# shanghong/Multiband-RF-pulse-Design

Hardware: AMD Instinct MI355X
Metric: FIR designs/sec, n=512 taps m=16384 arbitrary-phase SOCP (fir_ap_cvx form) (higher is better)
Workload: dtype f64

## Files before the change

include/mbfir.h:

```cpp
#ifndef MBFIR_H
#define MBFIR_H

#ifdef __cplusplus
extern "C" {
#endif

#define MBFIR_SOLVED 0
#define MBFIR_INFEASIBLE 1
#define MBFIR_NUMERICAL 2
#define MBFIR_EARLY_FAIL 3
#define MBFIR_E_ARG (-1)
#define MBFIR_E_HIP (-2)
#define MBFIR_E_NODEVICE (-3)

typedef struct mbfir_ctx mbfir_ctx;

typedef struct mbfir_opts {
    int grid_m;
    int max_iter;
    double feastol;
    double abstol;
    double reltol;
    int refine;
    int verbose;
// ... 21 lines not shown
    double chol_flop;
    int chol_launches;
    int builds;
    int dd_iters;
    int dd_kmax;
    int collectives;
    int lanes;
    int dd_form;
    double ms_cap;
    double cap_flop;
    double collective_bytes;
    int correctors;
    int correctors_taken;
    int gv_passes;
    int gtv_passes;
} mbfir_info;

typedef int (*mbfir_allreduce_fn)(void* buf, long count, int op, void* user);

int  mbfir_comm_unique_id(mbfir_ctx* ctx, char* id128);
int  mbfir_comm_init(mbfir_ctx* ctx, int nranks, int rank, const char* id128);
void mbfir_comm_destroy(mbfir_ctx* ctx);
int  mbfir_test_comm_allreduce(mbfir_ctx* ctx, double* v, long n, int op);

mbfir_ctx*  mbfir_create(int device_id);
void        mbfir_destroy(mbfir_ctx* ctx);
const char* mbfir_last_error(mbfir_ctx* ctx);
void        mbfir_default_opts(mbfir_opts* opts);
void        mbfir_set_allreduce(mbfir_ctx* ctx, mbfir_allreduce_fn fn, void* user);
const char* mbfir_version(void);
// ... 121 lines not shown
```

multiband-rf-pulse-design_amd/__init__.py:

```python
import ctypes as C
import os

import numpy as np

_HERE = os.path.dirname(os.path.abspath(__file__))
LIB_PATH = os.path.join(_HERE, "libmbfir.so")

SOLVED, INFEASIBLE, NUMERICAL, EARLY_FAIL = 0, 1, 2, 3
E_ARG, E_HIP, E_NODEVICE = -1, -2, -3


class MbfirError(RuntimeError):
    pass


class Opts(C.Structure):
    _fields_ = [("grid_m", C.c_int), ("max_iter", C.c_int), ("feastol", C.c_double),
                ("abstol", C.c_double), ("reltol", C.c_double), ("refine", C.c_int),
                ("verbose", C.c_int), ("shard_rank", C.c_int), ("shard_size", C.c_int),
                ("dense_trig", C.c_int), ("ddkkt", C.c_int), ("lanes", C.c_int)]


class Info(C.Structure):
    _fields_ = [("status", C.c_int), ("iters", C.c_int), ("n_unknowns", C.c_int), ("n_rows", C.c_int),
                ("n_freq", C.c_int), ("n_lp", C.c_int), ("n_q3", C.c_int), ("n_big", C.c_int),
                ("pcost", C.c_double), ("dcost", C.c_double), ("gap", C.c_double), ("relgap", C.c_double),
                ("pres", C.c_double), ("dres", C.c_double),
                ("ms_assemble", C.c_double), ("ms_solve", C.c_double), ("ms_post", C.c_double),
                ("ms_total", C.c_double), ("ms_gram", C.c_double), ("ms_chol", C.c_double),
                ("gram_flop", C.c_double), ("gram_launches", C.c_int), ("lattice", C.c_int),
                ("chol_flop", C.c_double), ("chol_launches", C.c_int), ("builds", C.c_int),
                ("dd_iters", C.c_int), ("dd_kmax", C.c_int), ("collectives", C.c_int), ("lanes", C.c_int),
                ("dd_form", C.c_int), ("ms_cap", C.c_double), ("cap_flop", C.c_double),
                ("collective_bytes", C.c_double), ("correctors", C.c_int), ("correctors_taken", C.c_int),
                ("gv_passes", C.c_int), ("gtv_passes", C.c_int)]

    def as_dict(self):
        return {k: getattr(self, k) for k, _ in self._fields_}


class Job(C.Structure):
    _fields_ = [("which", C.c_int), ("n", C.c_int), ("nband", C.c_int), ("rc", C.c_int),
                ("f", C.POINTER(C.c_double)), ("a", C.POINTER(C.c_double)), ("d", C.POINTER(C.c_double)),
                ("params", C.c_double * 4), ("h_re", C.POINTER(C.c_double)), ("h_im", C.POINTER(C.c_double)),
                ("info", Info), ("z", C.POINTER(C.c_double)), ("z_cap", C.c_int), ("err", C.c_char * 128)]


class RemezJob(C.Structure):
    _fields_ = [("numtaps", C.c_int), ("nband", C.c_int), ("type", C.c_int), ("edges", C.POINTER(C.c_double)),
                ("desired", C.POINTER(C.c_double)), ("weight", C.POINTER(C.c_double)), ("h", C.POINTER(C.c_double)),
# ... 1005 lines not shown
```

multiband-rf-pulse-design_amd/csrc/api.cpp:

```cpp
#include "../../include/mbfir.h"
#include "program.h"
#include "pulse.h"
#include "solver.h"
#include <chrono>
#include <cmath>
#include <cstdio>
#include <algorithm>
#include <cstdlib>
#include <cstring>
#include <functional>
#include <atomic>
#include <condition_variable>
#include <map>
#include <mutex>
#include <memory>
#include <system_error>
#include <thread>

using namespace mbfir;

struct mbfir_ctx {
    std::unique_ptr<Solver> solver;
    int device = 0;
    std::vector<double> last_x;
// ... 49 lines not shown
    info->status = rc; info->iters = si.iters; info->n_unknowns = P.N();
    info->n_rows = si.n_rows; info->n_freq = si.n_freq;
    info->n_lp = P.l; info->n_q3 = P.nq3; info->n_big = P.big;
    info->pcost = si.pcost; info->dcost = si.dcost; info->gap = si.gap; info->relgap = si.relgap;
    info->pres = si.pres; info->dres = si.dres;
    info->ms_assemble = (t_asm - t0) + si.ms_assemble; info->ms_solve = si.ms_solve;
    info->ms_post = t_end - t_solved; info->ms_total = t_end - t0;
    info->ms_gram = si.ms_gram; info->ms_chol = si.ms_chol; info->gram_flop = si.gram_flop;
    info->gram_launches = si.lattice ? 0 : si.h_builds * (P.quad ? 3 : 1);
    info->lattice = si.lattice;
    info->chol_launches = si.chol_launches; info->chol_flop = si.chol_flop; info->builds = si.h_builds;
    info->dd_iters = si.dd_iters; info->dd_kmax = si.dd_kmax; info->lanes = si.lanes; info->collectives = si.collectives;
    info->collective_bytes = si.collective_bytes;
    info->ms_cap = si.ms_cap; info->cap_flop = si.cap_flop; info->dd_form = si.dd_iters > 0 ? si.dd_form : -1;
    info->correctors = si.correctors; info->correctors_taken = si.correctors_taken; info->gv_passes = si.gv_passes; info->gtv_passes = si.gtv_passes;
}

void taps_from_solution(Solver& solver, const TrigProgram& P, const std::vector<double>& x, int lane, double* h_re, double* h_im) {
    const int n = P.n;
    switch (P.which) {
        case DES_AP:
            solver.specfact_last(n, h_re, h_im, lane);
            break;
        case DES_LINPROG: {
            const int nh = P.nhalf;
            for (int i = 0; i < n; ++i) { h_re[i] = 0; h_im[i] = 0; }
            if (P.real_filter) {
                if (P.odd_filter) for (int k = 0; k < nh; ++k) { h_re[nh - 1 + k] = x[k]; h_re[nh - 1 - k] = x[k]; }
                else for (int k = 0; k < nh; ++k) { h_re[nh + k] = x[k]; h_re[nh - 1 - k] = x[k]; }
            } else if (P.odd_filter) {
// ... 757 lines not shown
```

multiband-rf-pulse-design_amd/csrc/solver.h:

```cpp
#pragma once
#include "program.h"
#include <stdexcept>
#include <string>
#include <vector>

namespace mbfir {

struct ShapeError : std::runtime_error {
    explicit ShapeError(const std::string& s) : std::runtime_error(s) {}
};
struct ResourceError : std::runtime_error {
    explicit ResourceError(const std::string& s) : std::runtime_error(s) {}
};

enum { ST_OPTIMAL = 0, ST_PRIMAL_INFEASIBLE = 1, ST_DUAL_INFEASIBLE = 2, ST_MAXIT = 3, ST_NUMERICAL = 4,
       ST_OPTIMAL_INACCURATE = 5 };

struct SolveOpts {
    int max_iter = 200;
    double feastol = 1e-8, abstol = 1e-10, reltol = 1e-8;
    int refine = 2;
    int verbose = 0;
    int shard_rank = 0, shard_size = 1;
    bool dense_trig = false;
// ... 5 lines not shown
struct SolveInfo {
    int status = 0, iters = 0, n_unknowns = 0, n_rows = 0, n_freq = 0;
    double pcost = 0, dcost = 0, gap = 0, relgap = 0, pres = 0, dres = 0;
    double ms_assemble = 0, ms_solve = 0, ms_gram = 0, ms_chol = 0, gram_flop = 0;
    int h_builds = 0;
    int chol_launches = 0;
    double chol_flop = 0;
    int dd_iters = 0, dd_kmax = 0;
    double ms_cap = 0, cap_flop = 0;
    int dd_form = 0;
    int collectives = 0;
    double collective_bytes = 0;
    int lanes = 1;
    int lattice = 0;
    int correctors = 0, correctors_taken = 0;
    int gv_passes = 0, gtv_passes = 0;
};

class Solver {
public:
    explicit Solver(int device);
    ~Solver();
    Solver(const Solver&) = delete;
    Solver& operator=(const Solver&) = delete;
    int solve(const TrigProgram& P, const SolveOpts& o, std::vector<double>& xout, SolveInfo& info);
    void solve_lanes(const std::vector<const TrigProgram*>& Ps, const SolveOpts& o, std::vector<std::vector<double>>& xouts,
                     std::vector<SolveInfo>& infos);
    static std::vector<long> shape_key(const TrigProgram& P, const SolveOpts& o);
    static int max_lanes(const TrigProgram& P, const SolveOpts& o);
    static void test_fold(const double* w, int Mf, int fold, long* out);
// ... 24 lines not shown
```

multiband-rf-pulse-design_amd/csrc/solver.hip:

```cpp
#include "dev_common.h"
#include <functional>
#include <mutex>
#include <thread>
#include "cone_dev.h"
#include "dd_dev.h"
#include "program.h"
#include "solver.h"
#include <algorithm>
#include <chrono>
#include <cmath>
#include <cstdlib>
#include <cstring>
#include <vector>

#include <dlfcn.h>
#include <rccl/rccl.h>

namespace mbfir {

struct RcclApi {
    ncclResult_t (*GetUniqueId)(ncclUniqueId*) = nullptr;
    ncclResult_t (*CommInitRank)(ncclComm_t*, int, ncclUniqueId, int) = nullptr;
    ncclResult_t (*CommDestroy)(ncclComm_t) = nullptr;
    ncclResult_t (*AllReduce)(const void*, void*, size_t, ncclDataType_t, ncclRedOp_t, ncclComm_t, hipStream_t) = nullptr;
// ... 443 lines not shown
            if (P.own)
            for (int q = P.c_ptr[j]; q < P.c_ptr[j + 1]; ++q) {
                const int r = P.c_rows[q];
                g += P.alpha[r] * val[(long)v * P.Rp + r];
            }
            if (F.bx) __hip_atomic_store(out + (long)v * P.LDV + j, g, __ATOMIC_RELAXED, __HIP_MEMORY_SCOPE_AGENT);
            else out[(long)v * P.LDV + j] = g;
        }
    }
    if (F.bx) gt_resid_tail<NV>(P, F, out, red);
}

constexpr int CHK = 64;

constexpr int SEGMAX = 128;
template <int NV>
__global__ __launch_bounds__(256) void k_trig_eval(DProg P, const double* __restrict__ vin, double* __restrict__ UU) {
    LANES(P, vin, UU);
    constexpr int NVVMAX = 2 * NV;
    __shared__ double2 cf[NVVMAX][SEGMAX];
    const int k = blockIdx.x * 256 + threadIdx.x, sg = blockIdx.y;
    const int m0 = sg * P.seg, m1 = min(m0 + P.seg, P.D1);
    const int NVV = P.quad ? 2 * NV : NV;
    for (int e = threadIdx.x; e < 2 * (m1 - m0); e += 256) {
        const int kind = e & 1, m = m0 + (e >> 1), le = kind * P.D1 + m;
        const int j = P.lat_col[le], qj = P.quad ? P.lat_qcol[le] : -1;
        const double sc = P.lat_scale[le], qs = P.quad ? P.lat_qscale[le] : 0.0;
#pragma unroll
        for (int q = 0; q < NV; ++q) {
            const double c1 = j >= 0 ? sc * vin[(long)q * P.LDV + j] : 0.0;
            if (kind) cf[q][e >> 1].y = c1; else cf[q][e >> 1].x = c1;
            if (P.quad) {
                const double c2 = qj >= 0 ? qs * vin[(long)q * P.LDV + qj] : 0.0;
                if (kind) cf[NV + q][e >> 1].y = c2; else cf[NV + q][e >> 1].x = c2;
            }
        }
    }
    __syncthreads();
    if (k >= P.nfold) return;
    const double4 sd4 = P.seed_eval[(long)sg * P.Mpad + k];
    double c = sd4.x, s = sd4.y;
    const double cw = sd4.z, sw = sd4.w;
    double ac[NVVMAX], as[NVVMAX];
#pragma unroll
    for (int v = 0; v < NVVMAX; ++v) ac[v] = as[v] = 0;
#pragma unroll 8
    for (int m = 0; m < m1 - m0; ++m) {
#pragma unroll
        for (int v = 0; v < NVVMAX; ++v)
            if (v < NVV) { const double2 x = cf[v][m]; ac[v] += x.x * c; as[v] += x.y * s; }
        const double cn = c * cw - s * sw;
        s = s * cw + c * sw;
        c = cn;
    }
    const int ip = P.fold_pos[k], in = P.fold_neg[k];
#pragma unroll
    for (int v = 0; v < NVVMAX; ++v)
        if (v < NVV) {
            double* u = UU + ((long)sg * NVV + v) * P.Mpad;
            if (ip >= 0) u[ip] = ac[v] + as[v];
            if (in >= 0) u[in] = ac[v] - as[v];
        }
}

__global__ void k_build_seeds_m(DProg P, double ka, int na, double kb, int nb, double4* __restrict__ seeds) {
    LANES(P, seeds);
    if (P.dims) { na = P.D1; nb = nb ? 2 * P.D1 - 1 : 0; }
    const double t0a = ka * P.tmin, t0b = kb * P.tmin;
    const int m = blockIdx.x * blockDim.x + threadIdx.x, ch = blockIdx.y;
    if (m >= na + nb || ch >= P.nchunk) return;
    const double t = m < na ? t0a + m : t0b + (m - na);
    double s, c, sd, cd;
    sincos(P.ch_w0[ch] * t, &s, &c);
    sincos(P.ch_dw[ch] * t, &sd, &cd);
    seeds[(long)ch * (na + nb) + m] = make_double4(c, s, cd, sd);
}
__global__ void k_build_seeds_e(DProg P, double4* __restrict__ seeds) {
    LANES(P, seeds);
    const int i = blockIdx.x * blockDim.x + threadIdx.x, sg = blockIdx.y;
    if (i >= P.nfold) return;
    const double w = P.wf[i];
    double s, c, sw, cw;
    sincos(w * (P.tmin + sg * P.seg), &s, &c);
    sincos(w, &sw, &cw);
    seeds[(long)sg * P.Mpad + i] = make_double4(c, s, cw, sw);
}

constexpr int CGRP = 4;
constexpr int MPTS = 256;
template <int NV, bool AGG>
__device__ __forceinline__ void freq_operands(const DProg& P, const double* __restrict__ src, int i, double (&out)[NV]) {
#pragma unroll
    for (int v = 0; v < NV; ++v) out[v] = 0;
    if (i < 0) return;
    if (AGG) {
        const int nv = P.quad ? NV / 2 : NV;
        for (int qq = P.f_ptr[i]; qq < P.f_ptr[i + 1]; ++qq) {
            const int r = P.f_rows[qq];
            const double al = P.alpha[r], be = P.beta[r];
#pragma unroll
            for (int v = 0; v < NV; ++v)
                if (v < nv) {
                    const double x = src[(long)v * P.Rp + r];
                    out[v] += al * x;
// ... 4 lines not shown
#pragma unroll
        for (int v = 0; v < NV; ++v) out[v] = src[(long)v * P.Mpad + i];
    }
}
template <int NV, bool AGG>
__global__ __launch_bounds__(256) void k_freq_fold(DProg P, const double* __restrict__ src, double2* __restrict__ out) {
    LANES(P, src, out);
    const int k = blockIdx.x * 256 + threadIdx.x;
    if (k >= P.nfold) return;
    double a[NV], b[NV];
    freq_operands<NV, AGG>(P, src, P.fold_pos[k], a);
    freq_operands<NV, AGG>(P, src, P.fold_neg[k], b);
#pragma unroll
    for (int v = 0; v < NV; ++v) out[(long)v * P.Mpad + k] = make_double2(a[v] + b[v], a[v] - b[v]);
}
template <int NV, bool FOLD = false>
__global__ __launch_bounds__(256) void k_trig_moments(DProg P, const double2* __restrict__ src, const double4* __restrict__ seeds,
                                                      int na, int nb, double* __restrict__ partial, const double* __restrict__ rows = nullptr) {
    if (!P.seeds_shared && blockIdx.z) seeds = reinterpret_cast<const double4*>(reinterpret_cast<const char*>(seeds) + (size_t)blockIdx.z * P.lane_bytes);
    LANES(P, src, partial, rows);
    if (P.dims) { na = P.D1; nb = nb ? 2 * P.D1 - 1 : 0; }
    __shared__ double2 pp[NV][CGRP][CHK];
    const int tid = threadIdx.x;
    const int ch0 = blockIdx.y * P.cgrp;
    for (int e = tid; e < P.cgrp * CHK; e += 256) {
        const int cc = e / CHK, q = e - cc * CHK, ch = ch0 + cc;
        const bool live = ch < P.nchunk && q < P.ch_count[ch < P.nchunk ? ch : 0];
        const int k = live ? P.ch_start[ch] + q : 0;
        if constexpr (FOLD) {
            double a[NV], b[NV];
            freq_operands<NV, true>(P, rows, live ? P.fold_pos[k] : -1, a);
            freq_operands<NV, true>(P, rows, live ? P.fold_neg[k] : -1, b);
#pragma unroll
            for (int v = 0; v < NV; ++v) pp[v][cc][q] = make_double2(a[v] + b[v], a[v] - b[v]);
        } else {
#pragma unroll
        for (int v = 0; v < NV; ++v) pp[v][cc][q] = live ? src[(long)v * P.Mpad + k] : make_double2(0.0, 0.0);
        }
    }
    __syncthreads();
    const int m = blockIdx.x * MPTS + tid;
    if (m >= na + nb) return;
    double ag[NV], as[NV];
#pragma unroll
    for (int v = 0; v < NV; ++v) ag[v] = as[v] = 0;
    for (int cl = 0; cl < P.cgrp; cl += 2) {
        const int cha = ch0 + cl, chb = cha + 1;
        if (cha >= P.nchunk) break;
        const bool two = cl + 1 < P.cgrp && chb < P.nchunk;
        const double4 sa = seeds[(long)cha * (na + nb) + m];
        const double4 sb = two ? seeds[(long)chb * (na + nb) + m] : make_double4(0.0, 0.0, 0.0, 0.0);
        double c0 = sa.x, s0 = sa.y, c1 = sb.x, s1 = sb.y;
        const int cnt = max(P.ch_count[cha], two ? P.ch_count[chb] : 0);
        const int clb = two ? cl + 1 : cl;
#pragma unroll 4
        for (int q = 0; q < cnt; ++q) {
#pragma unroll
            for (int v = 0; v < NV; ++v) {
                const double2 pa = pp[v][cl][q], pb = pp[v][clb][q];
                ag[v] += pa.x * c0; as[v] += pa.y * s0;
                ag[v] += pb.x * c1; as[v] += pb.y * s1;
            }
            const double n0 = c0 * sa.z - s0 * sa.w, n1 = c1 * sb.z - s1 * sb.w;
            s0 = s0 * sa.z + c0 * sa.w; s1 = s1 * sb.z + c1 * sb.w;
            c0 = n0; c1 = n1;
        }
    }
#pragma unroll
    for (int v = 0; v < NV; ++v) {
        partial[(((long)blockIdx.y * NV + v) * 2) * P.LDM + m] = ag[v];
        partial[(((long)blockIdx.y * NV + v) * 2 + 1) * P.LDM + m] = as[v];
    }
}

template <int NC>
__device__ __forceinline__ void block_partials(double vals[NC], double* __restrict__ part, bool is_max) {
    __shared__ double sh[17];
#pragma unroll
    for (int c = 0; c < NC; ++c) {
        double s = is_max ? block_max(vals[c], sh) : block_sum(vals[c], sh);
        if (threadIdx.x == 0) part[(long)blockIdx.x * NC + c] = s;
    }
}
__device__ __forceinline__ double fold_partials(const double* part, int nb, int nc, int c, bool is_max, double* sh) {
    double a = is_max ? -1e300 : 0.0;
    for (int b = threadIdx.x; b < nb; b += blockDim.x) {
// ... 1156 lines not shown
    bool corr_big = true;
    int test_cap_kp = 0;
    int ar_chunks = 0;
    int ar_overlap = 1;
    int cgrp = 4;
    int ddform = -1;
    bool dd_blockinv = true;
    bool hsolve = true;
    bool fuse = true;
    bool speculate = true;
    bool trace_host = false;
    int fold = -1;
    int chol_split = -1;
    bool poison = false;
    int test_lose_flag = -1;
};
static SolveSwitches read_switches() {
    SolveSwitches w;
    auto flag = [](const char* name, bool& v) { if (const char* ev = std::getenv(name)) v = std::atoi(ev) != 0; };
    auto number = [](const char* name, int& v) { if (const char* ev = std::getenv(name)) v = std::atoi(ev); };
    flag("MBFIR_CORRECTOR", w.corrector); flag("MBFIR_CORR_BIG", w.corr_big); flag("MBFIR_DD_BLOCKINV", w.dd_blockinv);
    flag("MBFIR_HSOLVE", w.hsolve); flag("MBFIR_FUSE", w.fuse); flag("MBFIR_SPECULATE", w.speculate); flag("MBFIR_POISON", w.poison);
    number("MBFIR_TEST_CAP_KP", w.test_cap_kp); number("MBFIR_AR_OVERLAP", w.ar_overlap);
    number("MBFIR_CHOL_SPLIT", w.chol_split); number("MBFIR_TEST_LOSE_FLAG", w.test_lose_flag);
    if (const char* ev = std::getenv("MBFIR_CGRP")) w.cgrp = std::max(1, std::min(CGRP, std::atoi(ev)));
    if (const char* ev = std::getenv("MBFIR_AR_CHUNKS")) w.ar_chunks = std::max(1, std::atoi(ev));
    if (const char* ev = std::getenv("MBFIR_DDFORM")) w.ddform = std::strcmp(ev, "dd") != 0 ? 1 : 0;
    if (const char* ev = std::getenv("MBFIR_FOLD")) w.fold = std::atoi(ev) != 0;
    w.trace_host = std::getenv("MBFIR_TRACE_HOST") != nullptr;
    return w;
}

struct LatticeInfo {
    bool ok = false;
    double tmin = 0;
    int D1 = 0;
    std::vector<int> lat, lat_col, lat_qcol, ch_start, ch_count;
    std::vector<double> lat_scale, lat_qscale, ch_w0, ch_dw;
    std::vector<int> fold_pos, fold_neg;
    std::vector<double> wf;
};
constexpr int CHUNK_LEN = 64;
static_assert(CHUNK_LEN <= CHK, "a chunk holds at most CHK frequencies");
// ... 216 lines not shown
    if (L.wall >= WALL_ITERS) return finish(ST_NUMERICAL);
    return best;
}

struct Solver::Impl {
    int device = 0;
    hipStream_t st = nullptr;
    int shard_rank = 0, shard_size = 1;
    int (*ar_fn)(void*, long, int, void*) = nullptr;
    void* ar_user = nullptr;
    double* RB = nullptr;
    ncclComm_t comm = nullptr;
    int comm_size = 0, comm_rank = 0;
    long n_collectives = 0;
    double collective_bytes = 0;
    long n_gv = 0, n_gtv = 0;
    void allreduce(double* buf, long count, int op, hipStream_t on = nullptr) {
        if (shard_size <= 1) return;
        if (!on) on = st;
        ++n_collectives;
        collective_bytes += 8.0 * double(count);
        if (comm) {
            ncclResult_t r = rccl().AllReduce(buf, buf, size_t(count), ncclDouble, op == 1 ? ncclMax : ncclSum, comm, on);
            if (r != ncclSuccess) throw HipError(std::string("ncclAllReduce: ") + (rccl().GetErrorString ? rccl().GetErrorString(r) : "failed"));
            return;
        }
        MBFIR_HIP(hipStreamSynchronize(on));
        if (!ar_fn || ar_fn(buf, count, op, ar_user) != 0) throw HipError("all-reduce hook failed");
    }
    hipEvent_t ev0 = nullptr, ev1 = nullptr;
// ... 122 lines not shown
        pend.clear();
        stage_lo = stage_hi = 0;
    }
    void memset_lanes(void* p, size_t bytes) {
        if ((bytes & 15) == 0 && (reinterpret_cast<size_t>(p) & 15) == 0 && (lane_bytes & 15) == 0)
            hipLaunchKernelGGL(k_zero_lanes, dim3(std::min<size_t>(2048, cdiv((long)(bytes / 16), 256)), nlanes), dim3(256), 0, st,
                               reinterpret_cast<double2*>(p), bytes / 16, lane_bytes);
        else if (nlanes > 1) hipMemset2DAsync(p, lane_bytes, 0, bytes, nlanes, st);
        else hipMemsetAsync(p, 0, bytes, st);
    }
    void copy_lanes(void* dst, const void* src, size_t bytes) {
        if (nlanes > 1) MBFIR_HIP(hipMemcpy2DAsync(dst, lane_bytes, src, lane_bytes, bytes, nlanes, hipMemcpyDeviceToDevice, st));
        else MBFIR_HIP(hipMemcpyAsync(dst, src, bytes, hipMemcpyDeviceToDevice, st));
    }

    template <int NV>
    void apply_G(const double* v, double* out) {
        const int NVV = P.quad ? 2 * NV : NV;
        ++n_gv;
        if (P.trig) {
            hipLaunchKernelGGL(k_trig_eval<NV>, lane_grid(dim3(cdiv(P.nfold, 256), P.useg), nlanes), dim3(256), 0, st, P, v, UU);
            hipLaunchKernelGGL(k_rows_G<NV>, lane_grid(dim3(cdiv(P.R, 256)), nlanes), dim3(256), 0, st, P, UU, v, out);
            return;
        }
        const double* xx = v;
        if (P.quad) {
            hipLaunchKernelGGL(k_make_xx<NV>, lane_grid(dim3(cdiv(P.Nt, 256)), nlanes), dim3(256), 0, st, P, v, XX);
            xx = XX;
        }
        dim3 g(cdiv(P.Mf, 4));
        if (NVV == 1) hipLaunchKernelGGL(k_amulti<1>, lane_grid(g, nlanes), dim3(256), 0, st, A1, P.ld, P.Mf, xx, P.LDV, UU, P.Mpad, lane_bytes, P.mask, P.dims);
        else if (NVV == 2) hipLaunchKernelGGL(k_amulti<2>, lane_grid(g, nlanes), dim3(256), 0, st, A1, P.ld, P.Mf, xx, P.LDV, UU, P.Mpad, lane_bytes, P.mask, P.dims);
        else hipLaunchKernelGGL(k_amulti<4>, lane_grid(g, nlanes), dim3(256), 0, st, A1, P.ld, P.Mf, xx, P.LDV, UU, P.Mpad, lane_bytes, P.mask, P.dims);
        hipLaunchKernelGGL(k_rows_G<NV>, lane_grid(dim3(cdiv(P.R, 256)), nlanes), dim3(256), 0, st, P, UU, v, out);
    }
    template <int NV>
    void apply_G_winv2(const double* v, double* gout, const double* sub, double* wout) {
        if (P.trig && !P.big) {
            ++n_gv;
            hipLaunchKernelGGL(k_trig_eval<NV>, lane_grid(dim3(cdiv(P.nfold, 256), P.useg), nlanes), dim3(256), 0, st, P, v, UU);
            hipLaunchKernelGGL(k_rows_winv2<NV>, lane_grid(dim3(cdiv(P.l + P.nq3, 256)), nlanes), dim3(256), 0, st, P, UU, v, dl, w3, sub, gout, wout);
            return;
        }
        apply_G<NV>(v, gout);
        winv2<NV>(gout, sub, wout, 0);
    }
    void moments_array(int nv, const double* pp, const double4* seeds, int na, int nb, double* out) {
        dim3 g(cdiv(na + nb, MPTS), cdiv(P.nchunk, P.cgrp)), b(256), gf(cdiv(P.nfold, 256));
        switch (nv) {
#define MOM_CASE(NVX)                                                                                                          \
            case NVX:                                                                                                          \
                if (pp) hipLaunchKernelGGL((k_freq_fold<NVX, false>), lane_grid(gf, nlanes), b, 0, st, P, pp, PPf);            \
                hipLaunchKernelGGL((k_trig_moments<NVX>), lane_grid(g, nlanes), b, 0, st, P, PPf, seeds, na, nb, partial);     \
                break;
            MOM_CASE(1) MOM_CASE(2) MOM_CASE(3) MOM_CASE(4) MOM_CASE(6)
#undef MOM_CASE
            default: throw HipError("moments: unsupported vector count");
        }
        hipLaunchKernelGGL(k_fold_partials, lane_grid(dim3(cdiv(P.LDM, 64), 2 * nv), nlanes), dim3(64, 16), 0, st, partial, cdiv(P.nchunk, P.cgrp), 2 * nv, P.LDM, P.LDM, out, lane_bytes, P.mask, P.dims, P.cgrp);
    }
    void atmulti_array(int nvv, const double* pp) {
        dim3 g(P.ld / 128, nsplit_at), b(64, 4);
        switch (nvv) {
            case 1: hipLaunchKernelGGL((k_atmulti<1, false>), lane_grid(g, nlanes), b, 0, st, P, A1, pp, partial); break;
            case 2: hipLaunchKernelGGL((k_atmulti<2, false>), lane_grid(g, nlanes), b, 0, st, P, A1, pp, partial); break;
            case 3: hipLaunchKernelGGL((k_atmulti<3, false>), lane_grid(g, nlanes), b, 0, st, P, A1, pp, partial); break;
            case 4: hipLaunchKernelGGL((k_atmulti<4, false>), lane_grid(g, nlanes), b, 0, st, P, A1, pp, partial); break;
            case 6: hipLaunchKernelGGL((k_atmulti<6, false>), lane_grid(g, nlanes), b, 0, st, P, A1, pp, partial); break;
            default: throw HipError("atmulti: unsupported vector count");
        }
    }
    template <int NV>
    void apply_GT(const double* val, double* out, int tail = 0, const double* rn_bx = nullptr, double* rn_r = nullptr, int rn_slot = 0) {
        ++n_gtv;
        if (P.trig) {
            dim3 g(cdiv(P.D1, MPTS), cdiv(P.nchunk, P.cgrp)), b(256);
            const dim3 gf(cdiv(P.nfold, 256));
            if (sw.fuse) {
                if (P.quad) hipLaunchKernelGGL((k_trig_moments<2 * NV, true>), lane_grid(g, nlanes), b, 0, st, P, (const double2*)nullptr, P.seed_tau, P.D1, 0, partial, val);
                else hipLaunchKernelGGL((k_trig_moments<NV, true>), lane_grid(g, nlanes), b, 0, st, P, (const double2*)nullptr, P.seed_tau, P.D1, 0, partial, val);
            } else if (P.quad) {
                hipLaunchKernelGGL((k_freq_fold<2 * NV, true>), lane_grid(gf, nlanes), b, 0, st, P, val, PPf);
                hipLaunchKernelGGL((k_trig_moments<2 * NV>), lane_grid(g, nlanes), b, 0, st, P, PPf, P.seed_tau, P.D1, 0, partial);
            } else {
                hipLaunchKernelGGL((k_freq_fold<NV, true>), lane_grid(gf, nlanes), b, 0, st, P, val, PPf);
                hipLaunchKernelGGL((k_trig_moments<NV>), lane_grid(g, nlanes), b, 0, st, P, PPf, P.seed_tau, P.D1, 0, partial);
            }
        } else {
            dim3 g(P.ld / 128, nsplit_at), b(64, 4);
            if (P.quad) hipLaunchKernelGGL((k_atmulti<2 * NV, true>), lane_grid(g, nlanes), b, 0, st, P, A1, val, partial);
            else hipLaunchKernelGGL((k_atmulti<NV, true>), lane_grid(g, nlanes), b, 0, st, P, A1, val, partial);
        }
        hipLaunchKernelGGL(k_gt_finish<NV>, lane_grid(dim3(cdiv(P.Nt, GTC) + 1), nlanes), dim3(GTC, GTG), 0, st, P, partial, P.trig ? cdiv(P.nchunk, P.cgrp) : nsplit_at, val, out,
                           GtResid{rn_bx, rn_r, Sc, rn_slot, gt_cnt});
        allreduce(out, (long)NV * P.LDV + tail, 0);
    }
    template <int NV>
    void winv2(const double* in, const double* sub, double* out, int mode) {
        hipLaunchKernelGGL(k_winv2<NV>, lane_grid(dim3(cdiv(P.l + P.nq3, 256)), nlanes), dim3(256), 0, st, P, dl, w3, in, sub, out, mode);
        if (P.big) hipLaunchKernelGGL(k_big_winv2<NV>, lane_grid(dim3(1), nlanes), dim3(1024), 0, st, P, wbb, Sc, in, sub, out, mode);
    }
// ... 302 lines not shown
            hipLaunchKernelGGL(k_dd_rows, lane_grid(dim3(ddk), nlanes), dim3(256), 0, st, P, D, P.np, ddk);
            dd_syrk_launch(D.U, P.np, D.sX, D.kcnt, P.np, H, M, st);
            dd_chol_launch(H, M, Mt, W1, ddri, ddri + P.np, ddd0, P.np, DD_PIVTOL, flag, st, ddinv);
            if (c1) hipEventRecord(c1, st);
        } else {
            chol_launch_count += chol_inv_launch(H, M, fused_hsolve ? nullptr : Mt, W1, P.np, flag, st, sw.chol_split, sw.poison, nullptr, c0, c1, nlanes, lane_bytes, P.mask);
        }
    }
    void prepare_lanes(const std::vector<const TrigProgram*>& Qs, const SolveOpts& o, std::vector<LaneHost>& LH) {
        shard_rank = o.shard_size > 1 ? o.shard_rank : 0;
        shard_size = o.shard_size > 1 ? o.shard_size : 1;
        if (shard_size > 1 && !ar_fn && !comm) throw HipError("row-sharded solve without a communicator or an all-reduce hook");
        if (comm && shard_size > 1 && (comm_size != shard_size || comm_rank != shard_rank))
            throw HipError("row-sharded solve: shard_rank / shard_size differ from the RCCL communicator's");
        n_collectives = 0; collective_bytes = 0;
        n_gv = 0; n_gtv = 0;
        if (shard_size > 1 && nlanes > 1) throw ShapeError("row-sharded solves run one design at a time");
        for (int b = 0; b < nlanes; ++b) {
            LaneHost& L = LH[b];
            const TrigProgram& Qfull = *Qs[b];
            if (shard_size > 1) { L.local = shard_program(Qfull, shard_rank, shard_size); L.Q = &L.local; }
            else L.Q = &Qfull;
            double nh = 0, nc = 0;
            for (double v : Qfull.h) nh += v * v;
            for (double v : Qfull.c) nc += v * v;
            L.nrm_h = std::max(1.0, std::sqrt(nh)); L.nrm_c = std::max(1.0, std::sqrt(nc));
            L.degree = double(Qfull.l + Qfull.nq3 + (Qfull.big ? 1 : 0));
            L.prep = lane_prep(*L.Q, o, sw);
            L.Lt = L.prep->Lt;
            L.nsweep = o.refine; L.nsweep_ctl = o.refine;
        }
// ... 242 lines not shown
                           P, dl, wl, w3, wbb, Sc);
        build_H();
        hipLaunchKernelGGL(k_init_rhs, lane_grid(dim3(cdiv(std::max(P.N, P.R), 256)), nlanes), dim3(256), 0, st, P, bx2, bz2);
        kkt_solve<2>(bx2, bz2, dx2, dz2, gdx2, nsweep, S_RNA);
        copy_lanes(x, dx2, sizeof(double) * P.LDV);
        hipLaunchKernelGGL(k_neg_copy_r, lane_grid(dim3(cdiv(P.R, 256)), nlanes), dim3(256), 0, st, P, dz2, s, -1.0);
        cone_shift(s);
        hipLaunchKernelGGL(k_neg_copy_r, lane_grid(dim3(cdiv(P.R, 256)), nlanes), dim3(256), 0, st, P, dz2 + P.Rp, z, 1.0);
        cone_shift(z);
    }
    void launch_residuals() {
        const bool sharded = shard_size > 1;
        double* rmail = sharded ? GTz + P.LDV : RB;
        if (P.trig) {
            ++n_gv;
            hipLaunchKernelGGL(k_trig_eval<1>, lane_grid(dim3(cdiv(P.nfold, 256), P.useg), nlanes), dim3(256), 0, st, P, x, UU);
            hipLaunchKernelGGL(k_resid_rows, lane_grid(dim3(nbR), nlanes), dim3(256), 0, st, P, nullptr, s, z, Sc, rz, bz2, partR, UU, x);
        } else {
            apply_G<1>(x, Gx);
            hipLaunchKernelGGL(k_resid_rows, lane_grid(dim3(nbR), nlanes), dim3(256), 0, st, P, Gx, s, z, Sc, rz, bz2, partR, nullptr, nullptr);
        }
        if (sharded) hipLaunchKernelGGL(k_scal_resid, dim3(1), dim3(SCAL_T), 0, st, P, Sc, GTz, x, rx, bx2, partR, nbR, rmail, 0, (const int*)flag);
        apply_GT<1>(z, GTz, sharded ? 5 : 0);
        hipLaunchKernelGGL(k_scal_resid, lane_grid(dim3(1), nlanes), dim3(SCAL_T), 0, st, P, Sc, GTz, x, rx, bx2, partR, nbR, rmail, sharded ? 1 : 2, (const int*)flag);
    }
    void launch_head(std::vector<LaneHost>& LH, const SolveOpts& o) {
        hipLaunchKernelGGL(k_scaling, lane_grid(dim3(std::max(nbC, 1)), nlanes), dim3(256), 0, st, P, s, z, dl, wl, w3, lam, bz2, wbz);
        if (P.big) hipLaunchKernelGGL(k_big_scaling, lane_grid(dim3(1), nlanes), dim3(1024), 0, st, P, s, z, wbb, lam, Sc);
        int ks[MAX_LANES];
        if (dd_unit) {
            bool lv[MAX_LANES];
// ... 168 lines not shown
        for (size_t i = 0; i + 1 < capev_used; i += 2) { float t = 0; hipEventElapsedTime(&t, capev[i], capev[i + 1]); ms_cap += t; }
        const int nw = P.quad ? 3 : 1;
        for (int b = 0; b < nlanes; ++b) {
            SolveInfo& info = infos[b];
            info = LH[b].info;
            info.status = LH[b].status;
            info.ms_assemble = t_assembled - t_begin;
            info.ms_solve = t_end - t_assembled;
            info.ms_gram = ms_gram; info.ms_chol = ms_chol; info.h_builds = builds;
            info.n_freq = LH[b].Q->Mf; info.n_rows = LH[b].Q->R; info.n_unknowns = LH[b].Q->N();
            info.lattice = P.trig;
            info.lanes = nlanes;
            info.collectives = int(n_collectives);
            info.collective_bytes = collective_bytes;
            info.gv_passes = int(n_gv); info.gtv_passes = int(n_gtv);
            info.dd_iters = LH[b].dd_iters; info.dd_kmax = LH[b].dd_kmax;
            info.dd_form = cap_form ? 0 : 1; info.cap_flop = cap_flop_sum; info.ms_cap = ms_cap;
            info.chol_launches = int(chol_launch_count);
            info.chol_flop = 2.0 / 3.0 * double(P.np) * double(P.np) * double(P.np);
            info.gram_flop = P.trig ? double(3 * P.D1 - 1) * double(LH[b].Q->Mf) * (4.0 + 4.0 * nw)
                                    : double(nw) * double(P.Mf) * double(P.Nt) * double(P.Nt + 1);
        }
        nlanes_last = nlanes; taps_valid = false;
    }
};

Solver::Solver(int device) : impl(new Impl()) {
    impl->device = device;
    int ndev = 0;
    if (hipGetDeviceCount(&ndev) != hipSuccess || ndev <= 0) throw HipError("no HIP device available");
// ... 505 lines not shown
```

Measured before the change: 300.5.

## Block multiple lanes per workgroup in trig eval and moment kernels

Adds lane-blocked variants of the trig evaluation and trig moment kernels so one workgroup handles several batched designs. The shared seed rotation (cos/sin recurrence) is computed once and reused across lanes, and the moments kernel picks a smaller block size when there are too few blocks to fill the CUs. It also pins FMA contraction so results stay bit-consistent with the per-lane path. In exchange it uses more shared memory and registers per block, which can lower occupancy. It only takes effect when several lanes run with shared seeds.

```diff
diff --git a/include/mbfir.h b/include/mbfir.h
--- a/include/mbfir.h
+++ b/include/mbfir.h
@@ -59,6 +59,9 @@
     int correctors_taken;
     int gv_passes;
     int gtv_passes;
+    int lb_gv_passes;
+    int lb_gtv_passes;
+    int lb_moment_launches;
 } mbfir_info;
 
 typedef int (*mbfir_allreduce_fn)(void* buf, long count, int op, void* user);
diff --git a/multiband-rf-pulse-design_amd/__init__.py b/multiband-rf-pulse-design_amd/__init__.py
--- a/multiband-rf-pulse-design_amd/__init__.py
+++ b/multiband-rf-pulse-design_amd/__init__.py
@@ -33,7 +33,8 @@
                 ("dd_iters", C.c_int), ("dd_kmax", C.c_int), ("collectives", C.c_int), ("lanes", C.c_int),
                 ("dd_form", C.c_int), ("ms_cap", C.c_double), ("cap_flop", C.c_double),
                 ("collective_bytes", C.c_double), ("correctors", C.c_int), ("correctors_taken", C.c_int),
-                ("gv_passes", C.c_int), ("gtv_passes", C.c_int)]
+                ("gv_passes", C.c_int), ("gtv_passes", C.c_int),
+                ("lb_gv_passes", C.c_int), ("lb_gtv_passes", C.c_int), ("lb_moment_launches", C.c_int)]
 
     def as_dict(self):
         return {k: getattr(self, k) for k, _ in self._fields_}
diff --git a/multiband-rf-pulse-design_amd/csrc/api.cpp b/multiband-rf-pulse-design_amd/csrc/api.cpp
--- a/multiband-rf-pulse-design_amd/csrc/api.cpp
+++ b/multiband-rf-pulse-design_amd/csrc/api.cpp
@@ -87,6 +87,7 @@
     info->collective_bytes = si.collective_bytes;
     info->ms_cap = si.ms_cap; info->cap_flop = si.cap_flop; info->dd_form = si.dd_iters > 0 ? si.dd_form : -1;
     info->correctors = si.correctors; info->correctors_taken = si.correctors_taken; info->gv_passes = si.gv_passes; info->gtv_passes = si.gtv_passes;
+    info->lb_gv_passes = si.lb_gv_passes; info->lb_gtv_passes = si.lb_gtv_passes; info->lb_moment_launches = si.lb_moment_launches;
 }
 
 void taps_from_solution(Solver& solver, const TrigProgram& P, const std::vector<double>& x, int lane, double* h_re, double* h_im) {
diff --git a/multiband-rf-pulse-design_amd/csrc/solver.h b/multiband-rf-pulse-design_amd/csrc/solver.h
--- a/multiband-rf-pulse-design_amd/csrc/solver.h
+++ b/multiband-rf-pulse-design_amd/csrc/solver.h
@@ -43,6 +43,7 @@
     int lanes = 1;
     int lattice = 0;
     int correctors = 0, correctors_taken = 0;
+    int lb_gv_passes = 0, lb_gtv_passes = 0, lb_moment_launches = 0;
     int gv_passes = 0, gtv_passes = 0;
 };
 
diff --git a/multiband-rf-pulse-design_amd/csrc/solver.hip b/multiband-rf-pulse-design_amd/csrc/solver.hip
--- a/multiband-rf-pulse-design_amd/csrc/solver.hip
+++ b/multiband-rf-pulse-design_amd/csrc/solver.hip
@@ -481,25 +481,65 @@
 constexpr int CHK = 64;
 
 constexpr int SEGMAX = 128;
-template <int NV>
-__global__ __launch_bounds__(256) void k_trig_eval(DProg P, const double* __restrict__ vin, double* __restrict__ UU) {
-    LANES(P, vin, UU);
+template <bool EVAL>
+__device__ __forceinline__ void trig_rot(double& c, double& s, double cd, double sd) {
+#pragma clang fp contract(off)
+    const double n = fma(c, cd, -(s * sd));
+    s = EVAL ? fma(s, cd, c * sd) : fma(c, sd, s * cd);
+    c = n;
+}
+__device__ __forceinline__ void trig_acc(double& acc, double p, double t) {
+#pragma clang fp contract(off)
+    acc = fma(p, t, acc);
+}
+template <int LB>
+__device__ __forceinline__ bool lane_group(const DProg& P, int nlanes, bool (&on)[LB]) {
+    bool any = false;
+#pragma unroll
+    for (int l = 0; l < LB; ++l) {
+        const int lane = blockIdx.z * LB + l;
+        on[l] = lane < nlanes && (!P.mask || P.mask[lane]);
+        any = any || on[l];
+    }
+    return any;
+}
+template <int NV, int LB = 1>
+__global__ __launch_bounds__(256) void k_trig_eval(DProg P, const double* __restrict__ vin, double* __restrict__ UU, int nlanes = 1) {
+    bool on[LB];
+    if constexpr (LB == 1) {
+        LANES(P, vin, UU);
+        on[0] = true;
+    } else if (!lane_group<LB>(P, nlanes, on)) return;
     constexpr int NVVMAX = 2 * NV;
-    __shared__ double2 cf[NVVMAX][SEGMAX];
+    __shared__ double2 cf[LB][NVVMAX][SEGMAX];
     const int k = blockIdx.x * 256 + threadIdx.x, sg = blockIdx.y;
     const int m0 = sg * P.seg, m1 = min(m0 + P.seg, P.D1);
     const int NVV = P.quad ? 2 * NV : NV;
-    for (int e = threadIdx.x; e < 2 * (m1 - m0); e += 256) {
-        const int kind = e & 1, m = m0 + (e >> 1), le = kind * P.D1 + m;
-        const int j = P.lat_col[le], qj = P.quad ? P.lat_qcol[le] : -1;
-        const double sc = P.lat_scale[le], qs = P.quad ? P.lat_qscale[le] : 0.0;
-#pragma unroll
-        for (int q = 0; q < NV; ++q) {
-            const double c1 = j >= 0 ? sc * vin[(long)q * P.LDV + j] : 0.0;
-            if (kind) cf[q][e >> 1].y = c1; else cf[q][e >> 1].x = c1;
-            if (P.quad) {
-                const double c2 = qj >= 0 ? qs * vin[(long)q * P.LDV + qj] : 0.0;
-                if (kind) cf[NV + q][e >> 1].y = c2; else cf[NV + q][e >> 1].x = c2;
+#pragma unroll
+    for (int l = 0; l < LB; ++l) {
+        DProg Q = P;
+        const double* vl = vin;
+        if constexpr (LB > 1) {
+            const size_t off = (size_t)(blockIdx.z * LB + l) * P.lane_bytes;
+            if (on[l] && off) { Q.shift(off); lane_shift(off, vl); }
+        }
+        for (int e = threadIdx.x; e < 2 * (m1 - m0); e += 256) {
+            const int kind = e & 1, m = m0 + (e >> 1), le = kind * P.D1 + m;
+            if (LB > 1 && !on[l]) {
+#pragma unroll
+                for (int q = 0; q < NVVMAX; ++q) { if (kind) cf[l][q][e >> 1].y = 0.0; else cf[l][q][e >> 1].x = 0.0; }
+                continue;
+            }
+            const int j = Q.lat_col[le], qj = P.quad ? Q.lat_qcol[le] : -1;
+            const double sc = Q.lat_scale[le], qs = P.quad ? Q.lat_qscale[le] : 0.0;
+#pragma unroll
+            for (int q = 0; q < NV; ++q) {
+                const double c1 = j >= 0 ? sc * vl[(long)q * P.LDV + j] : 0.0;
+                if (kind) cf[l][q][e >> 1].y = c1; else cf[l][q][e >> 1].x = c1;
+                if (P.quad) {
+                    const double c2 = qj >= 0 ? qs * vl[(long)q * P.LDV + qj] : 0.0;
+                    if (kind) cf[l][NV + q][e >> 1].y = c2; else cf[l][NV + q][e >> 1].x = c2;
+                }
             }
         }
     }
@@ -508,26 +548,37 @@
     const double4 sd4 = P.seed_eval[(long)sg * P.Mpad + k];
     double c = sd4.x, s = sd4.y;
     const double cw = sd4.z, sw = sd4.w;
-    double ac[NVVMAX], as[NVVMAX];
-#pragma unroll
-    for (int v = 0; v < NVVMAX; ++v) ac[v] = as[v] = 0;
-#pragma unroll 8
+    double ac[LB][NVVMAX], as[LB][NVVMAX];
+#pragma unroll
+    for (int l = 0; l < LB; ++l)
+#pragma unroll
+        for (int v = 0; v < NVVMAX; ++v) ac[l][v] = as[l][v] = 0;
+    constexpr int UNR = LB >= 4 ? 4 : 8;
+#pragma unroll UNR
     for (int m = 0; m < m1 - m0; ++m) {
 #pragma unroll
+        for (int l = 0; l < LB; ++l)
+#pragma unroll
+            for (int v = 0; v < NVVMAX; ++v)
+                if (v < NVV) { const double2 x = cf[l][v][m]; trig_acc(ac[l][v], x.x, c); trig_acc(as[l][v], x.y, s); }
+        trig_rot<true>(c, s, cw, sw);
+    }
+#pragma unroll
+    for (int l = 0; l < LB; ++l) {
+        if (LB > 1 && !on[l]) continue;
+        const size_t off = LB > 1 ? (size_t)(blockIdx.z * LB + l) * P.lane_bytes : 0;
+        DProg Q = P;
+        double* ul = UU;
+        if (off) { Q.shift(off); lane_shift(off, ul); }
+        const int ip = Q.fold_pos[k], in = Q.fold_neg[k];
+#pragma unroll
         for (int v = 0; v < NVVMAX; ++v)
-            if (v < NVV) { const double2 x = cf[v][m]; ac[v] += x.x * c; as[v] += x.y * s; }
-        const double cn = c * cw - s * sw;
-        s = s * cw + c * sw;
-        c = cn;
-    }
-    const int ip = P.fold_pos[k], in = P.fold_neg[k];
-#pragma unroll
-    for (int v = 0; v < NVVMAX; ++v)
-        if (v < NVV) {
-            double* u = UU + ((long)sg * NVV + v) * P.Mpad;
-            if (ip >= 0) u[ip] = ac[v] + as[v];
-            if (in >= 0) u[in] = ac[v] - as[v];
-        }
+            if (v < NVV) {
+                double* u = ul + ((long)sg * NVV + v) * P.Mpad;
+                if (ip >= 0) u[ip] = ac[l][v] + as[l][v];
+                if (in >= 0) u[in] = ac[l][v] - as[l][v];
+            }
+    }
 }
 
 __global__ void k_build_seeds_m(DProg P, double ka, int na, double kb, int nb, double4* __restrict__ seeds) {
@@ -555,6 +606,7 @@
 
 constexpr int CGRP = 4;
 constexpr int MPTS = 256;
+constexpr int NUM_CU = 256;
 template <int NV, bool AGG>
 __device__ __forceinline__ void freq_operands(const DProg& P, const double* __restrict__ src, int i, double (&out)[NV]) {
 #pragma unroll
@@ -589,36 +641,54 @@
 #pragma unroll
     for (int v = 0; v < NV; ++v) out[(long)v * P.Mpad + k] = make_double2(a[v] + b[v], a[v] - b[v]);
 }
-template <int NV, bool FOLD = false>
-__global__ __launch_bounds__(256) void k_trig_moments(DProg P, const double2* __restrict__ src, const double4* __restrict__ seeds,
-                                                      int na, int nb, double* __restrict__ partial, const double* __restrict__ rows = nullptr) {
-    if (!P.seeds_shared && blockIdx.z) seeds = reinterpret_cast<const double4*>(reinterpret_cast<const char*>(seeds) + (size_t)blockIdx.z * P.lane_bytes);
-    LANES(P, src, partial, rows);
-    if (P.dims) { na = P.D1; nb = nb ? 2 * P.D1 - 1 : 0; }
-    __shared__ double2 pp[NV][CGRP][CHK];
+template <int NV, bool FOLD = false, int LB = 1, int MP = MPTS>
+__global__ __launch_bounds__(MP) void k_trig_moments(DProg P, const double2* __restrict__ src, const double4* __restrict__ seeds,
+                                                     int na, int nb, double* __restrict__ partial, const double* __restrict__ rows = nullptr,
+                                                     int nlanes = 1) {
+    bool on[LB];
+    if constexpr (LB == 1) {
+        if (!P.seeds_shared && blockIdx.z) seeds = reinterpret_cast<const double4*>(reinterpret_cast<const char*>(seeds) + (size_t)blockIdx.z * P.lane_bytes);
+        LANES(P, src, partial, rows);
+        if (P.dims) { na = P.D1; nb = nb ? 2 * P.D1 - 1 : 0; }
+        on[0] = true;
+    } else if (!lane_group<LB>(P, nlanes, on)) return;
+    __shared__ double2 pp[LB][NV][CGRP][CHK];
     const int tid = threadIdx.x;
     const int ch0 = blockIdx.y * P.cgrp;
-    for (int e = tid; e < P.cgrp * CHK; e += 256) {
-        const int cc = e / CHK, q = e - cc * CHK, ch = ch0 + cc;
-        const bool live = ch < P.nchunk && q < P.ch_count[ch < P.nchunk ? ch : 0];
-        const int k = live ? P.ch_start[ch] + q : 0;
-        if constexpr (FOLD) {
-            double a[NV], b[NV];
-            freq_operands<NV, true>(P, rows, live ? P.fold_pos[k] : -1, a);
-            freq_operands<NV, true>(P, rows, live ? P.fold_neg[k] : -1, b);
-#pragma unroll
-            for (int v = 0; v < NV; ++v) pp[v][cc][q] = make_double2(a[v] + b[v], a[v] - b[v]);
-        } else {
-#pragma unroll
-        for (int v = 0; v < NV; ++v) pp[v][cc][q] = live ? src[(long)v * P.Mpad + k] : make_double2(0.0, 0.0);
+#pragma unroll
+    for (int l = 0; l < LB; ++l) {
+        DProg Q = P;
+        const double2* srcl = src;
+        const double* rowsl = rows;
+        if constexpr (LB > 1) {
+            const size_t off = (size_t)(blockIdx.z * LB + l) * P.lane_bytes;
+            if (on[l] && off) { Q.shift(off); lane_shift(off, srcl, rowsl); }
+        }
+        for (int e = tid; e < P.cgrp * CHK; e += MP) {
+            const int cc = e / CHK, q = e - cc * CHK, ch = ch0 + cc;
+            const bool live = (LB == 1 || on[l]) && ch < P.nchunk && q < Q.ch_count[ch < P.nchunk ? ch : 0];
+            const int k = live ? Q.ch_start[ch] + q : 0;
+            if constexpr (FOLD) {
+                double a[NV], b[NV];
+                freq_operands<NV, true>(Q, rowsl, live ? Q.fold_pos[k] : -1, a);
+                freq_operands<NV, true>(Q, rowsl, live ? Q.fold_neg[k] : -1, b);
+#pragma unroll
+                for (int v = 0; v < NV; ++v) pp[l][v][cc][q] = make_double2(a[v] + b[v], a[v] - b[v]);
+            } else {
+#pragma unroll
+                for (int v = 0; v < NV; ++v) pp[l][v][cc][q] = live ? srcl[(long)v * P.Mpad + k] : make_double2(0.0, 0.0);
+            }
         }
     }
     __syncthreads();
-    const int m = blockIdx.x * MPTS + tid;
+    const int m = blockIdx.x * MP + tid;
     if (m >= na + nb) return;
-    double ag[NV], as[NV];
-#pragma unroll
-    for (int v = 0; v < NV; ++v) ag[v] = as[v] = 0;
+    constexpr int UNR = LB * NV >= 4 && LB > 1 ? 2 : 4;
+    double ag[LB][NV], as[LB][NV];
+#pragma unroll
+    for (int l = 0; l < LB; ++l)
+#pragma unroll
+        for (int v = 0; v < NV; ++v) ag[l][v] = as[l][v] = 0;
     for (int cl = 0; cl < P.cgrp; cl += 2) {
         const int cha = ch0 + cl, chb = cha + 1;
         if (cha >= P.nchunk) break;
@@ -628,23 +698,30 @@
         double c0 = sa.x, s0 = sa.y, c1 = sb.x, s1 = sb.y;
         const int cnt = max(P.ch_count[cha], two ? P.ch_count[chb] : 0);
         const int clb = two ? cl + 1 : cl;
-#pragma unroll 4
+#pragma unroll UNR
         for (int q = 0; q < cnt; ++q) {
 #pragma unroll
-            for (int v = 0; v < NV; ++v) {
-                const double2 pa = pp[v][cl][q], pb = pp[v][clb][q];
-                ag[v] += pa.x * c0; as[v] += pa.y * s0;
-                ag[v] += pb.x * c1; as[v] += pb.y * s1;
-            }
-            const double n0 = c0 * sa.z - s0 * sa.w, n1 = c1 * sb.z - s1 * sb.w;
-            s0 = s0 * sa.z + c0 * sa.w; s1 = s1 * sb.z + c1 * sb.w;
-            c0 = n0; c1 = n1;
-        }
-    }
-#pragma unroll
-    for (int v = 0; v < NV; ++v) {
-        partial[(((long)blockIdx.y * NV + v) * 2) * P.LDM + m] = ag[v];
-        partial[(((long)blockIdx.y * NV + v) * 2 + 1) * P.LDM + m] = as[v];
+            for (int l = 0; l < LB; ++l)
+#pragma unroll
+                for (int v = 0; v < NV; ++v) {
+                    const double2 pa = pp[l][v][cl][q], pb = pp[l][v][clb][q];
+                    trig_acc(ag[l][v], pa.x, c0); trig_acc(as[l][v], pa.y, s0);
+                    trig_acc(ag[l][v], pb.x, c1); trig_acc(as[l][v], pb.y, s1);
+                }
+            trig_rot<false>(c0, s0, sa.z, sa.w);
+            trig_rot<false>(c1, s1, sb.z, sb.w);
+        }
+    }
+#pragma unroll
+    for (int l = 0; l < LB; ++l) {
+        if (LB > 1 && !on[l]) continue;
+        double* pl = partial;
+        if constexpr (LB > 1) lane_shift((size_t)(blockIdx.z * LB + l) * P.lane_bytes, pl);
+#pragma unroll
+        for (int v = 0; v < NV; ++v) {
+            pl[(((long)blockIdx.y * NV + v) * 2) * P.LDM + m] = ag[l][v];
+            pl[(((long)blockIdx.y * NV + v) * 2 + 1) * P.LDM + m] = as[l][v];
+        }
     }
 }
 
@@ -1831,6 +1908,8 @@
     int chol_split = -1;
     bool poison = false;
     int test_lose_flag = -1;
+    int laneblk = 0;
+    int mpts = 0;
 };
 static SolveSwitches read_switches() {
     SolveSwitches w;
@@ -1844,6 +1923,8 @@
     if (const char* ev = std::getenv("MBFIR_AR_CHUNKS")) w.ar_chunks = std::max(1, std::atoi(ev));
     if (const char* ev = std::getenv("MBFIR_DDFORM")) w.ddform = std::strcmp(ev, "dd") != 0 ? 1 : 0;
     if (const char* ev = std::getenv("MBFIR_FOLD")) w.fold = std::atoi(ev) != 0;
+    if (const char* ev = std::getenv("MBFIR_LANEBLK")) { const int k = std::atoi(ev); w.laneblk = k >= 8 ? 8 : k >= 4 ? 4 : k >= 2 ? 2 : k == 1 ? 1 : 0; }
+    if (const char* ev = std::getenv("MBFIR_MPTS")) { const int k = std::atoi(ev); w.mpts = k == 64 || k == 128 || k == 256 ? k : 0; }
     w.trace_host = std::getenv("MBFIR_TRACE_HOST") != nullptr;
     return w;
 }
@@ -2090,6 +2171,7 @@
     int comm_size = 0, comm_rank = 0;
     long n_collectives = 0;
     double collective_bytes = 0;
+    long n_lb_gv = 0, n_lb_gtv = 0, n_lb_mom = 0;
     long n_gv = 0, n_gtv = 0;
     void allreduce(double* buf, long count, int op, hipStream_t on = nullptr) {
         if (shard_size <= 1) return;
@@ -2242,12 +2324,54 @@
         else MBFIR_HIP(hipMemcpyAsync(dst, src, bytes, hipMemcpyDeviceToDevice, st));
     }
 
+    static constexpr int lane_block_most(int nv) { return nv == 1 ? 8 : nv == 2 ? 4 : nv <= 4 ? 2 : 1; }
+    static constexpr int LANEBLK_AUTO = 4;
+    int lane_block(int most) const {
+        if (!P.trig || !P.seeds_shared || P.dims || nlanes <= 1 || sw.laneblk == 1) return 1;
+        int lb = 1;
+        while (lb < nlanes && lb < most) lb *= 2;
+        return std::min(lb, sw.laneblk > 1 ? sw.laneblk : LANEBLK_AUTO);
+    }
+    template <int NV>
+    void launch_trig_eval(const double* v) {
+        constexpr int MOST = lane_block_most(NV);
+        const dim3 g(cdiv(P.nfold, 256), P.useg), b(256);
+        const int lb = lane_block(MOST);
+        if (lb == 1) { hipLaunchKernelGGL((k_trig_eval<NV, 1>), lane_grid(g, nlanes), b, 0, st, P, v, UU, nlanes); return; }
+        ++n_lb_gv;
+#define EVAL_LB(LBX)                                                                                                                    \
+        if constexpr (LBX <= MOST) if (lb == LBX) hipLaunchKernelGGL((k_trig_eval<NV, LBX>), lane_grid(g, cdiv(nlanes, LBX)), b, 0, st, P, v, UU, nlanes);
+        EVAL_LB(2) EVAL_LB(4) EVAL_LB(8)
+#undef EVAL_LB
+    }
+    template <int NV, bool FOLD>
+    void launch_trig_moments(const double2* src, const double4* seeds, int na, int nb, const double* rows, long& blocked) {
+        constexpr int MOST = lane_block_most(NV);
+        const int lb = lane_block(MOST), npts = na + nb, groups = cdiv(P.nchunk, P.cgrp);
+        if (lb == 1) {
+            hipLaunchKernelGGL((k_trig_moments<NV, FOLD, 1, MPTS>), lane_grid(dim3(cdiv(npts, MPTS), groups), nlanes), dim3(MPTS), 0, st, P, src, seeds, na, nb, partial, rows, nlanes);
+            return;
+        }
+        ++blocked;
+        int mp = sw.mpts ? sw.mpts : MPTS;
+        if (!sw.mpts) while (mp > 64 && (mp / 2 >= npts || cdiv(npts, mp) * groups * cdiv(nlanes, lb) < NUM_CU)) mp /= 2;
+        const dim3 g(cdiv(npts, mp), groups, cdiv(nlanes, lb)), b(mp);
+#define MOM_LB(LBX)                                                                                                                     \
+        if constexpr (LBX <= MOST) if (lb == LBX) {                                                                                     \
+            if (mp == 64) hipLaunchKernelGGL((k_trig_moments<NV, FOLD, LBX, 64>), g, b, 0, st, P, src, seeds, na, nb, partial, rows, nlanes);        \
+            else if (mp == 128) hipLaunchKernelGGL((k_trig_moments<NV, FOLD, LBX, 128>), g, b, 0, st, P, src, seeds, na, nb, partial, rows, nlanes); \
+            else hipLaunchKernelGGL((k_trig_moments<NV, FOLD, LBX, 256>), g, b, 0, st, P, src, seeds, na, nb, partial, rows, nlanes);               \
+        }
+        MOM_LB(2) MOM_LB(4) MOM_LB(8)
+#undef MOM_LB
+    }
+
     template <int NV>
     void apply_G(const double* v, double* out) {
         const int NVV = P.quad ? 2 * NV : NV;
         ++n_gv;
         if (P.trig) {
-            hipLaunchKernelGGL(k_trig_eval<NV>, lane_grid(dim3(cdiv(P.nfold, 256), P.useg), nlanes), dim3(256), 0, st, P, v, UU);
+            launch_trig_eval<NV>(v);
             hipLaunchKernelGGL(k_rows_G<NV>, lane_grid(dim3(cdiv(P.R, 256)), nlanes), dim3(256), 0, st, P, UU, v, out);
             return;
         }
@@ -2266,7 +2390,7 @@
     void apply_G_winv2(const double* v, double* gout, const double* sub, double* wout) {
         if (P.trig && !P.big) {
             ++n_gv;
-            hipLaunchKernelGGL(k_trig_eval<NV>, lane_grid(dim3(cdiv(P.nfold, 256), P.useg), nlanes), dim3(256), 0, st, P, v, UU);
+            launch_trig_eval<NV>(v);
             hipLaunchKernelGGL(k_rows_winv2<NV>, lane_grid(dim3(cdiv(P.l + P.nq3, 256)), nlanes), dim3(256), 0, st, P, UU, v, dl, w3, sub, gout, wout);
             return;
         }
@@ -2274,12 +2398,12 @@
         winv2<NV>(gout, sub, wout, 0);
     }
     void moments_array(int nv, const double* pp, const double4* seeds, int na, int nb, double* out) {
-        dim3 g(cdiv(na + nb, MPTS), cdiv(P.nchunk, P.cgrp)), b(256), gf(cdiv(P.nfold, 256));
+        dim3 b(256), gf(cdiv(P.nfold, 256));
         switch (nv) {
 #define MOM_CASE(NVX)                                                                                                          \
             case NVX:                                                                                                          \
                 if (pp) hipLaunchKernelGGL((k_freq_fold<NVX, false>), lane_grid(gf, nlanes), b, 0, st, P, pp, PPf);            \
-                hipLaunchKernelGGL((k_trig_moments<NVX>), lane_grid(g, nlanes), b, 0, st, P, PPf, seeds, na, nb, partial);     \
+                launch_trig_moments<NVX, false>(PPf, seeds, na, nb, nullptr, n_lb_mom);                                        \
                 break;
             MOM_CASE(1) MOM_CASE(2) MOM_CASE(3) MOM_CASE(4) MOM_CASE(6)
 #undef MOM_CASE
@@ -2302,17 +2426,16 @@
     void apply_GT(const double* val, double* out, int tail = 0, const double* rn_bx = nullptr, double* rn_r = nullptr, int rn_slot = 0) {
         ++n_gtv;
         if (P.trig) {
-            dim3 g(cdiv(P.D1, MPTS), cdiv(P.nchunk, P.cgrp)), b(256);
-            const dim3 gf(cdiv(P.nfold, 256));
+            const dim3 gf(cdiv(P.nfold, 256)), b(256);
             if (sw.fuse) {
-                if (P.quad) hipLaunchKernelGGL((k_trig_moments<2 * NV, true>), lane_grid(g, nlanes), b, 0, st, P, (const double2*)nullptr, P.seed_tau, P.D1, 0, partial, val);
-                else hipLaunchKernelGGL((k_trig_moments<NV, true>), lane_grid(g, nlanes), b, 0, st, P, (const double2*)nullptr, P.seed_tau, P.D1, 0, partial, val);
+                if (P.quad) launch_trig_moments<2 * NV, true>(nullptr, P.seed_tau, P.D1, 0, val, n_lb_gtv);
+                else launch_trig_moments<NV, true>(nullptr, P.seed_tau, P.D1, 0, val, n_lb_gtv);
             } else if (P.quad) {
                 hipLaunchKernelGGL((k_freq_fold<2 * NV, true>), lane_grid(gf, nlanes), b, 0, st, P, val, PPf);
-                hipLaunchKernelGGL((k_trig_moments<2 * NV>), lane_grid(g, nlanes), b, 0, st, P, PPf, P.seed_tau, P.D1, 0, partial);
+                launch_trig_moments<2 * NV, false>(PPf, P.seed_tau, P.D1, 0, nullptr, n_lb_gtv);
             } else {
                 hipLaunchKernelGGL((k_freq_fold<NV, true>), lane_grid(gf, nlanes), b, 0, st, P, val, PPf);
-                hipLaunchKernelGGL((k_trig_moments<NV>), lane_grid(g, nlanes), b, 0, st, P, PPf, P.seed_tau, P.D1, 0, partial);
+                launch_trig_moments<NV, false>(PPf, P.seed_tau, P.D1, 0, nullptr, n_lb_gtv);
             }
         } else {
             dim3 g(P.ld / 128, nsplit_at), b(64, 4);
@@ -2645,7 +2768,7 @@
         if (comm && shard_size > 1 && (comm_size != shard_size || comm_rank != shard_rank))
             throw HipError("row-sharded solve: shard_rank / shard_size differ from the RCCL communicator's");
         n_collectives = 0; collective_bytes = 0;
-        n_gv = 0; n_gtv = 0;
+        n_gv = 0; n_gtv = 0; n_lb_gv = 0; n_lb_gtv = 0; n_lb_mom = 0;
         if (shard_size > 1 && nlanes > 1) throw ShapeError("row-sharded solves run one design at a time");
         for (int b = 0; b < nlanes; ++b) {
             LaneHost& L = LH[b];
@@ -2918,7 +3041,7 @@
         double* rmail = sharded ? GTz + P.LDV : RB;
         if (P.trig) {
             ++n_gv;
-            hipLaunchKernelGGL(k_trig_eval<1>, lane_grid(dim3(cdiv(P.nfold, 256), P.useg), nlanes), dim3(256), 0, st, P, x, UU);
+            launch_trig_eval<1>(x);
             hipLaunchKernelGGL(k_resid_rows, lane_grid(dim3(nbR), nlanes), dim3(256), 0, st, P, nullptr, s, z, Sc, rz, bz2, partR, UU, x);
         } else {
             apply_G<1>(x, Gx);
@@ -3117,6 +3240,7 @@
             info.collectives = int(n_collectives);
             info.collective_bytes = collective_bytes;
             info.gv_passes = int(n_gv); info.gtv_passes = int(n_gtv);
+            info.lb_gv_passes = int(n_lb_gv); info.lb_gtv_passes = int(n_lb_gtv); info.lb_moment_launches = int(n_lb_mom);
             info.dd_iters = LH[b].dd_iters; info.dd_kmax = LH[b].dd_kmax;
             info.dd_form = cap_form ? 0 : 1; info.cap_flop = cap_flop_sum; info.ms_cap = ms_cap;
             info.chol_launches = int(chol_launch_count);
```

New measurement: 289.4. 0.963x the previous value.
